# gabrielcheda/optimized-rag

Hardware: AMD Instinct MI355X
Metric: queries/sec + p50 retrieve+rerank latency, 1536-d top-k=20 (higher is better)
Workload: dtype f16 MFMA + block-scaled bf8 MFMA corrections (fp32 acc) in the cross-encoder; f16 MFMA pass + f64 rescore in the dense leg; f64 BM25 / RRF; 1 GPU; 1000000 docs x 1536-d + BM25 postings (2M-term Zipf vocabulary) + 224-token passage store; batch=256 queries: dense top-100 + BM25 top-100 + RRF -> top-100 -> ms-marco-MiniLM-L-6 cross-encoder (L=256, 25,600 pairs, seeded weights) -> top-20 (BASELINE.json configs[3]); corpus_rows=1000000, rows_per_gpu=1000000, batch_queries=256, pool=100, k=20, parallelism=one rag_retrieve_rerank_dev call per batch, exchange=single process

## Files before the change

### optimized-rag_amd/csrc/ce_mx.h

```cpp
#pragma once
#include "common.h"

typedef int mx_v8i __attribute__((ext_vector_type(8)));
typedef int mx_v4i __attribute__((ext_vector_type(4)));

#define MX_TM 384
#define MX_TN 128
#define MX_A_PLANE (MX_TM * 16)
#define MX_B_PLANE (MX_TN * 16)
#define MX_A_STAGE (6 * MX_A_PLANE)
#define MX_B_STAGE (6 * MX_B_PLANE)
#define MX_STAGE (MX_A_STAGE + MX_B_STAGE)
#define MX_STAGES 3
#define MX_LDS (MX_STAGES * MX_STAGE)
#ifndef MX_HI8_TRUNCATE
#define MX_LO_SCALE 2048.0f
#else
#define MX_LO_SCALE (2048.0f * 1.0928961748633879f)
#endif
#define MX_SCALE_A 116
#define MX_SCALE_B 127

__host__ __device__ __forceinline__ int mx_hi_off(int rows, int r, int e) {
    const int j = e >> 4, h = (e >> 2) & 1, i = ((e >> 3) & 1) * 4 + (e & 3);
// ... 258 lines not shown
    MX_STORE16(img + hh * MX_B_PLANE + trow * 16, ((mx_u4){hi[0][0], hi[0][1], hi[1][0], hi[1][1]}));
    MX_STORE16(img + (2 + hh) * MX_B_PLANE + trow * 16, ((mx_u4){hi[2][0], hi[2][1], hi[3][0], hi[3][1]}));
    MX_STORE16(img + (4 + hh) * MX_B_PLANE + trow * 16, ((mx_u4){lo[0], lo[2], lo[1], lo[3]}));
}

__global__ void mx_pack_weight_kernel(const float* __restrict__ w, int N, int K, char* __restrict__ out) {
    const int64_t i = (int64_t)blockIdx.x * blockDim.x + threadIdx.x;
    if (i >= (int64_t)N * K) return;
    const int n = (int)(i / K), k = (int)(i % K);
    const float x = w[i];
    const half_t hi = (half_t)x;
    const half_t l = (half_t)((x - (float)hi) * MX_LO_SCALE);
    char* img = out + ((size_t)(n / MX_TM) * (K >> 5) + (k >> 5)) * MX_A_STAGE;
    *reinterpret_cast<half_t*>(img + mx_hi_off(MX_TM, n % MX_TM, k & 31)) = hi;
    *reinterpret_cast<unsigned char*>(img + mx_lo_off(MX_TM, n % MX_TM, k & 31)) =
        (unsigned char)mx_e5m2_rn((unsigned)__builtin_bit_cast(unsigned short, l));
}

#define MX_EMB_ROWS 16
__global__ __launch_bounds__(256) void mx_embed_ln_kernel(const int32_t* __restrict__ ids, const int32_t* __restrict__ tt,
                                                           const float* __restrict__ word, const float* __restrict__ pos,
                                                           const float* __restrict__ type, const float* __restrict__ g,
                                                           const float* __restrict__ b, const int32_t* __restrict__ m_packed,
                                                           const int32_t* __restrict__ row_pair, const int32_t* __restrict__ pair_off,
                                                           int L, int vocab, float eps, char* __restrict__ x8) {
    constexpr int H = 384, NK = H / 32;
    __shared__ __attribute__((aligned(16))) char tile[NK * 6 * MX_EMB_ROWS * 16];
    const int lane = threadIdx.x & 63, wv = threadIdx.x >> 6;
    const int64_t base = (int64_t)blockIdx.x * MX_EMB_ROWS;
    const int n_rows = m_packed[0];
    if (base >= n_rows) return;
    const bool on = lane < H / 8;
    const int c = on ? lane : 0;
    const float4 g0 = *reinterpret_cast<const float4*>(g + c * 8), g1 = *reinterpret_cast<const float4*>(g + c * 8 + 4);
    const float4 b0 = *reinterpret_cast<const float4*>(b + c * 8), b1 = *reinterpret_cast<const float4*>(b + c * 8 + 4);
    const int j = (c >> 1) & 1, u = c & 1;
    char* const my = tile + (c >> 2) * 6 * MX_EMB_ROWS * 16;
#pragma unroll
    for (int r4 = 0; r4 < MX_EMB_ROWS / 4; ++r4) {
        const int rl = wv * (MX_EMB_ROWS / 4) + r4;
        const int64_t row = base + rl;
        if (row >= n_rows) break;
        const int pr = row_pair[row];
        const int p = (int)row - pair_off[pr];
        const size_t src = (size_t)pr * L + p;
        int id = ids[src];
        id = id < 0 ? 0 : (id >= vocab ? vocab - 1 : id);
        const int ty = tt[src] != 0;
        float v[8];
        {
            const float4* wp = reinterpret_cast<const float4*>(word + (size_t)id * H + c * 8);
            const float4* tp = reinterpret_cast<const float4*>(type + (size_t)ty * H + c * 8);
            const float4* pp = reinterpret_cast<const float4*>(pos + (size_t)p * H + c * 8);
#pragma unroll
            for (int q = 0; q < 2; ++q) {
                const float4 a = wp[q], t4 = tp[q], qq = pp[q];
                v[q * 4] = a.x + t4.x + qq.x; v[q * 4 + 1] = a.y + t4.y + qq.y; v[q * 4 + 2] = a.z + t4.z + qq.z; v[q * 4 + 3] = a.w + t4.w + qq.w;
            }
        }
        float s = 0.f;
#pragma unroll
        for (int i = 0; i < 8; ++i) s += on ? v[i] : 0.f;
#pragma unroll
        for (int o = 32; o > 0; o >>= 1) s += __shfl_xor(s, o);
        const float mean = s * (1.0f / H);
        float qd = 0.f;
#pragma unroll
// ... 4 lines not shown
        if (on) {
            mx_u2 h0, h1;
            unsigned l0, l1;
            mx_split4((v[0] - mean) * rstd * g0.x + b0.x, (v[1] - mean) * rstd * g0.y + b0.y, (v[2] - mean) * rstd * g0.z + b0.z,
                      (v[3] - mean) * rstd * g0.w + b0.w, h0, l0);
            mx_split4((v[4] - mean) * rstd * g1.x + b1.x, (v[5] - mean) * rstd * g1.y + b1.y, (v[6] - mean) * rstd * g1.z + b1.z,
                      (v[7] - mean) * rstd * g1.w + b1.w, h1, l1);
            char* o = my + rl * 16;
            *reinterpret_cast<mx_u2*>(o + (2 * j) * MX_EMB_ROWS * 16 + u * 8) = h0;
            *reinterpret_cast<mx_u2*>(o + (2 * j + 1) * MX_EMB_ROWS * 16 + u * 8) = h1;
            *reinterpret_cast<unsigned*>(o + 4 * MX_EMB_ROWS * 16 + u * 8 + j * 4) = l0;
            *reinterpret_cast<unsigned*>(o + 5 * MX_EMB_ROWS * 16 + u * 8 + j * 4) = l1;
        }
    }
    __syncthreads();
    const int trow0 = (int)(base & 127);
    char* const out = x8 + (size_t)(base >> 7) * NK * MX_B_STAGE + trow0 * 16;
    for (int i = threadIdx.x; i < NK * 6 * MX_EMB_ROWS; i += 256) {
        const int sp = i >> 4, r = i & (MX_EMB_ROWS - 1);
        if (base + r < n_rows) *reinterpret_cast<mx_u4*>(out + (size_t)sp * MX_B_PLANE + r * 16) = *reinterpret_cast<const mx_u4*>(tile + i * 16);
    }
}

__global__ void mx_gather_rows_kernel(const char* __restrict__ a, const char* __restrict__ b, const int32_t* __restrict__ pair_off, int P, int nk,
                                      char* __restrict__ a_out, char* __restrict__ b_out, int32_t* __restrict__ rows_out) {
    const int64_t i = (int64_t)blockIdx.x * blockDim.x + threadIdx.x;
    if (i == 0) rows_out[0] = P;
    const int per = nk * 6;
    if (i >= (int64_t)P * per) return;
    const int p = (int)(i / per), c = (int)(i % per), s = c / 6, pl = c % 6;
    const int64_t m = pair_off[p];
    const size_t src = ((size_t)(m >> 7) * nk + s) * MX_B_STAGE + (size_t)pl * MX_B_PLANE + (size_t)(m & 127) * 16;
    const size_t dst = ((size_t)(p >> 7) * nk + s) * MX_B_STAGE + (size_t)pl * MX_B_PLANE + (size_t)(p & 127) * 16;
    *reinterpret_cast<mx_u4*>(a_out + dst) = *reinterpret_cast<const mx_u4*>(a + src);
    if (b != nullptr) *reinterpret_cast<mx_u4*>(b_out + dst) = *reinterpret_cast<const mx_u4*>(b + src);
}

__device__ __forceinline__ float mx_load_elem(const char* __restrict__ x8, int64_t m, int k, int nk) {
    const char* img = x8 + mx_img_base(m, k, nk);
    const int trow = (int)(m & 127);
    return mx_join(*reinterpret_cast<const half_t*>(img + mx_hi_off(MX_TN, trow, k & 31)),
                   *reinterpret_cast<const unsigned char*>(img + mx_lo_off(MX_TN, trow, k & 31)));
}

struct mx_epi_qkv {
    half_t *qf16, *kf16, *vf16;
    size_t kv_plane;
    const float* bias;
    int m_tiles16;
    int ft_base;
    const int32_t* row_map;
    int n_map;
    __device__ __forceinline__ bool swap_for(int ft) const { return ft + ft_base == 2; }
    __device__ __forceinline__ void prepare(char* scratch) const { mx_stage_params(reinterpret_cast<float*>(scratch + MX_PARAM_OFF), bias, 3 * MX_TM); }
    __device__ __forceinline__ void operator()(f32x16 (&acc)[6], int tt, int ft_launch, bool swap, char* scratch) const {
        const float* const bias = reinterpret_cast<const float*>(scratch + MX_PARAM_OFF);
        const int ft = ft_launch + ft_base;
        const int lane = threadIdx.x & 63, wid = threadIdx.x >> 6, wm = wid >> 2, wn = wid & 3;
        const int li = lane & 31, hh = lane >> 5;
        const int m0 = tt * MX_TN + wn * 32;
        if (!swap) {
            half_t* dst = ft == 0 ? qf16 : kf16;
            int m = m0 + li;
            if (row_map != nullptr) {
                if (m >= n_map) return;
                m = row_map[m];
            }
#pragma unroll
            for (int b = 0; b < 6; ++b) {
                const int head = wm * 6 + b;
                half_t* tile = dst + (((size_t)head * m_tiles16 + (m >> 4)) * 64 + (m & 15)) * 8 + 4 * hh;
#pragma unroll
                for (int q = 0; q < 4; ++q) {
                    const float4 bv = *reinterpret_cast<const float4*>(bias + ft * MX_TM + head * 32 + 8 * q + 4 * hh);
                    const float v0 = acc[b][q * 4] + bv.x, v1 = acc[b][q * 4 + 1] + bv.y, v2 = acc[b][q * 4 + 2] + bv.z, v3 = acc[b][q * 4 + 3] + bv.w;
                    const half4 hi = {(half_t)v0, (half_t)v1, (half_t)v2, (half_t)v3};
                    const half4 lo = mx_resid4(hi, v0, v1, v2, v3);
                    __builtin_nontemporal_store(hi, reinterpret_cast<half4*>(tile + q * 128));
                    __builtin_nontemporal_store(lo, reinterpret_cast<half4*>(tile + q * 128 + kv_plane));
                }
            }
        } else {
#pragma unroll
            for (int b = 0; b < 6; ++b) {
                const int head = wm * 6 + b;
                const float bv = bias[2 * MX_TM + head * 32 + li];
#pragma unroll
                for (int q = 0; q < 4; ++q) {
                    const float v0 = acc[b][q * 4] + bv, v1 = acc[b][q * 4 + 1] + bv, v2 = acc[b][q * 4 + 2] + bv, v3 = acc[b][q * 4 + 3] + bv;
                    const half4 hi = {(half_t)v0, (half_t)v1, (half_t)v2, (half_t)v3};
                    const half4 lo = mx_resid4(hi, v0, v1, v2, v3);
                    half_t* o = vf16 + ((((size_t)head * m_tiles16 + (m0 >> 4) + (q >> 1)) * 2 + (li >> 4)) * 64 + (2 * (q & 1) + hh) * 16 + (li & 15)) * 4;
                    __builtin_nontemporal_store(hi, reinterpret_cast<half4*>(o));
                    __builtin_nontemporal_store(lo, reinterpret_cast<half4*>(o + kv_plane));
                }
            }
        }
    }
};

__device__ __forceinline__ float ce_gelu(float x) {
    const float z = fabsf(x) * 0.70710678118654752440f;
    const float t = __builtin_amdgcn_rcpf(fmaf(0.3275911f, z, 1.0f));
    float p = fmaf(1.061405429f, t, -1.453152027f);
    p = fmaf(p, t, 1.421413741f);
    p = fmaf(p, t, -0.284496736f);
    p = fmaf(p, t, 0.254829592f);
    const float e = __builtin_amdgcn_exp2f(-z * z * 1.4426950408889634f);
    const float erf_abs = fmaf(-p * t, e, 1.0f);
    return 0.5f * x * (1.0f + copysignf(erf_abs, x));
}
__device__ __forceinline__ float mx_gelu(float x) {
    const float z = fabsf(x) * 0.70710678118654752440f;
    const float t = __builtin_amdgcn_rcpf(fmaf(0.3275911f, z, 1.0f));
    float p = fmaf(1.061405429f, t, -1.453152027f);
// ... 123 lines not shown
```

### optimized-rag_amd/csrc/cross_encoder.hip

```cpp
#include "common.h"
#include "ce_mx.h"
#include <type_traits>

#include <cmath>
#include <cstdlib>
#include <cstring>

struct ce_chunk_bufs {
    dev_buf<int32_t> ids, tt, lens;
    dev_buf<int32_t> clen;
    dev_buf<int32_t> pair_off, row_pair, m_packed;
    dev_buf<int32_t> sid, stt;
    dev_buf<float> logits;
};

struct ce_ws_base {
    int pairs = 0, L = 0;
    int64_t tokens = 0;
    ce_chunk_bufs io;
    bool fits(int P, int L_) const { return P <= pairs && L_ == L; }
};
struct ce_split_ws : ce_ws_base {
    dev_buf<float> y32;
    dev_buf<half_t> x16, q16, kf16, vf16, ctx16, h16;
};
struct ce_mx_ws : ce_ws_base {
    dev_buf<char> x8, ctx8, h8;
    dev_buf<char> xc8, cc8, hc8;
    dev_buf<int32_t> m_cls;
    dev_buf<half_t> qf16, kf16, vf16;
};

struct ce_heads {
    int tok_dim = 0, tok_pad = 0;
// ... 302 lines not shown
                                               int hidden, float eps, int lane, half_t* __restrict__ o16) {
    float s = 0.f;
#pragma unroll
    for (int i = 0; i < PER; ++i) s += v[i];
#pragma unroll
    for (int o = 32; o > 0; o >>= 1) s += __shfl_xor(s, o);
    const float mean = s / (float)hidden;
    float q = 0.f;
#pragma unroll
    for (int i = 0; i < PER; ++i) { const float d = v[i] - mean; q += d * d; }
#pragma unroll
    for (int o = 32; o > 0; o >>= 1) q += __shfl_xor(q, o);
    const float rstd = 1.0f / sqrtf(q / (float)hidden + eps);
#pragma unroll
    for (int i = 0; i < PER; ++i) {
        const int c = lane + i * 64;
        const float y = (v[i] - mean) * rstd * g[c] + b[c];
        const half_t hi = (half_t)y;
        o16[SPLIT_IDX(c)] = hi;
        o16[SPLIT_IDX(c) + 32] = (half_t)(y - (float)hi);
    }
}

__global__ __launch_bounds__(1024) void ce_pack_scan_kernel(const int32_t* __restrict__ lens, int P, int L_in, int32_t* __restrict__ clen,
                                                             int32_t* __restrict__ pair_off, int32_t* __restrict__ m_packed) {
    __shared__ int part[1024];
    const int tid = threadIdx.x;
    const int per = (P + 1023) / 1024;
    const int b = tid * per, e = min(P, b + per);
    int s = 0;
    for (int p = b; p < e; ++p) s += (max(1, min(lens[p], L_in)) + 15) & ~15;
    part[tid] = s;
    __syncthreads();
    for (int o = 1; o < 1024; o <<= 1) {
        const int v = tid >= o ? part[tid - o] : 0;
        __syncthreads();
        part[tid] += v;
        __syncthreads();
    }
    int off = part[tid] - s;
    for (int p = b; p < e; ++p) {
        const int len = max(1, min(lens[p], L_in));
        clen[p] = len;
        pair_off[p] = off;
        off += (len + 15) & ~15;
    }
    if (tid == 1023) { pair_off[P] = part[1023]; m_packed[0] = part[1023]; }
}

__global__ void ce_pack_rows_kernel(const int32_t* __restrict__ pair_off, int P, int L, int64_t rows_total,
                                    int32_t* __restrict__ row_pair) {
    const int64_t i = (int64_t)blockIdx.x * blockDim.x + threadIdx.x;
    if (i < rows_total && i >= pair_off[P]) row_pair[i] = -1;
    if (i >= (int64_t)P * L) return;
    const int p = (int)(i / L), t = (int)(i % L);
    if (t < pair_off[p + 1] - pair_off[p]) row_pair[pair_off[p] + t] = p;
}

template <int PER>
__global__ __launch_bounds__(256) void ce_embed_ln_kernel(const int32_t* __restrict__ ids, const int32_t* __restrict__ tt,
                                                           const float* __restrict__ word, const float* __restrict__ pos,
                                                           const float* __restrict__ type, const float* __restrict__ g,
                                                           const float* __restrict__ b, const int32_t* __restrict__ m_packed,
                                                           const int32_t* __restrict__ row_pair, const int32_t* __restrict__ pair_off,
                                                           int L, int hidden, int vocab, int max_pos, float eps, half_t* __restrict__ x16) {
    const int lane = threadIdx.x & 63;
    const int64_t row = (int64_t)blockIdx.x * 4 + (threadIdx.x >> 6);
    if (row >= m_packed[0]) return;
    const int pr = row_pair[row];
    const int p = (int)row - pair_off[pr];
    const int pp = min(p, max_pos - 1);
    const size_t src = (size_t)pr * L + p;
    int id = ids[src];
    id = id < 0 ? 0 : (id >= vocab ? vocab - 1 : id);
    const int ty = tt[src] != 0;
    float v[PER];
#pragma unroll
    for (int i = 0; i < PER; ++i) {
        const int c = lane + i * 64;
// ... 12 lines not shown
    float v[PER];
#pragma unroll
    for (int i = 0; i < PER; ++i) v[i] = y32[tok * hidden + lane + i * 64];
    wave_layernorm<PER>(v, g, b, hidden, eps, lane, x16 + tok * 2 * hidden);
}

typedef uint32_t u32x4 __attribute__((ext_vector_type(4)));
typedef uint32_t u32x2 __attribute__((ext_vector_type(2)));
__device__ __forceinline__ uint32_t ce_pk(float a, float b) {
    return __builtin_bit_cast(uint32_t, __builtin_amdgcn_cvt_pkrtz(a, b));
}
__device__ __forceinline__ float ce_trunc10(float e) {
    return __builtin_bit_cast(float, __builtin_bit_cast(uint32_t, e) & 0xFFFFE000u);
}
__device__ __forceinline__ void ce_dma_at(const half_t* __restrict__ g, char* lds_uniform) {
    __builtin_amdgcn_global_load_lds((const __attribute__((address_space(1))) void*)g,
                                     (__attribute__((address_space(3))) void*)lds_uniform, 16, 0, 0);
}

template <int QB, bool MX = false, bool DIRECT = false>
__global__ __launch_bounds__(1024) void ce_attention_kernel(const half_t* __restrict__ q16,
                                                             const half_t* __restrict__ kf16, const half_t* __restrict__ vf16,
                                                             size_t kv_plane, const int32_t* __restrict__ lens,
                                                             const int32_t* __restrict__ pair_off, int L, int hidden,
                                                             int heads, int m_pad, half_t* __restrict__ ctx16, int max_qblocks = 1 << 20) {
    extern __shared__ __attribute__((aligned(16))) char smem[];
    const int lane = threadIdx.x & 63;
    const int wv = __builtin_amdgcn_readfirstlane(threadIdx.x >> 6), nwaves = blockDim.x >> 6;
    const int head = blockIdx.x, pair = blockIdx.y;
    const int len = max(1, min(lens[pair], L));
    const int fr = lane & 15, fq = lane >> 4;
    const int po = pair_off[pair], Lp = pair_off[pair + 1] - po;
    const int nt = Lp >> 4;
    const int nkb = (len + 31) >> 5;
    const size_t plane_b = (size_t)L * 64;
    const size_t t0 = ((size_t)head * (m_pad >> 4) + (po >> 4)) * 512;
    const char* const k_hi = DIRECT ? reinterpret_cast<const char*>(kf16 + t0) : smem;
    const char* const k_lo = DIRECT ? reinterpret_cast<const char*>(kf16 + t0 + kv_plane) : smem + plane_b;
    const char* const v_hi = DIRECT ? reinterpret_cast<const char*>(vf16 + t0) : smem + 2 * plane_b;
    const char* const v_lo = DIRECT ? reinterpret_cast<const char*>(vf16 + t0 + kv_plane) : smem + 3 * plane_b;
    if (!DIRECT) {
        char* const sk_hi = smem;
        char* const sk_lo = smem + plane_b;
        char* const sv_hi = smem + 2 * plane_b;
        char* const sv_lo = smem + 3 * plane_b;
        const size_t g0 = (((size_t)head * (m_pad >> 4) + (po >> 4)) * 64 + lane) * 8;
        for (int c = wv; c < nt; c += nwaves) {
            ce_dma_at(kf16 + g0 + (size_t)c * 512, sk_hi + c * 1024);
            ce_dma_at(kf16 + g0 + kv_plane + (size_t)c * 512, sk_lo + c * 1024);
            ce_dma_at(vf16 + g0 + (size_t)c * 512, sv_hi + c * 1024);
            ce_dma_at(vf16 + g0 + kv_plane + (size_t)c * 512, sv_lo + c * 1024);
        }
        if ((nt & 1) && wv == 0) {
            *reinterpret_cast<u32x4*>(sv_hi + nt * 1024 + lane * 16) = (u32x4){0u, 0u, 0u, 0u};
            *reinterpret_cast<u32x4*>(sv_lo + nt * 1024 + lane * 16) = (u32x4){0u, 0u, 0u, 0u};
// ... 8 lines not shown
        const int qb = (qb0 + b) * 16 < Lp ? qb0 + b : qb0;
        if (MX) {
            const half_t* qp = q16 + (((size_t)head * (m_pad >> 4) + (po >> 4) + qb) * 64 + lane) * 8;
            qh[b] = *reinterpret_cast<const half8*>(qp);
            ql[b] = *reinterpret_cast<const half8*>(qp + kv_plane);
        } else {
            const half_t* qp = q16 + (row0 + qb * 16 + fr) * (2 * hidden) + head * 64 + fq * 8;
            qh[b] = *reinterpret_cast<const half8*>(qp);
            ql[b] = *reinterpret_cast<const half8*>(qp + 32);
        }
    }
    f32x4 c0[QB], c1[QB];
    float mrun[QB], lsum[QB];
#pragma unroll
    for (int b = 0; b < QB; ++b) {
        c0[b] = (f32x4){0.f, 0.f, 0.f, 0.f};
        c1[b] = (f32x4){0.f, 0.f, 0.f, 0.f};
        mrun[b] = -INFINITY;
        lsum[b] = 0.f;
    }
    const float cs = (float)(0.17677669529663687 * 1.4426950408889634);
    if (!DIRECT) {
        asm volatile("s_waitcnt vmcnt(0)" ::: "memory");
        __syncthreads();
    }
    if (!has_rows) return;
    float ce_inf;
    asm volatile("s_mov_b32 %0, 0x7f800000" : "=s"(ce_inf));
#define CE_MAX2(a_, b_) __builtin_amdgcn_fmed3f(a_, b_, ce_inf)
    auto key_block = [&](const int kb, auto edge_c) {
        constexpr bool EDGE = decltype(edge_c)::value;
        const int fo = kb * 2048 + lane * 16;
        const half8 k0h = *reinterpret_cast<const half8*>(k_hi + fo), k1h = *reinterpret_cast<const half8*>(k_hi + fo + 1024);
        const half8 k0l = *reinterpret_cast<const half8*>(k_lo + fo), k1l = *reinterpret_cast<const half8*>(k_lo + fo + 1024);
        const int vo = kb * 2048 + lane * 8;
        const half4 a0h = *reinterpret_cast<const half4*>(v_hi + vo), a1h = *reinterpret_cast<const half4*>(v_hi + vo + 512);
        const half4 a0l = *reinterpret_cast<const half4*>(v_lo + vo), a1l = *reinterpret_cast<const half4*>(v_lo + vo + 512);
        half4 b0h = {}, b1h = {}, b0l = {}, b1l = {};
        if (!(DIRECT && EDGE && (nt & 1))) {
            b0h = *reinterpret_cast<const half4*>(v_hi + vo + 1024);
            b1h = *reinterpret_cast<const half4*>(v_hi + vo + 1536);
            b0l = *reinterpret_cast<const half4*>(v_lo + vo + 1024);
            b1l = *reinterpret_cast<const half4*>(v_lo + vo + 1536);
        }
        const half8 v0h = __builtin_shufflevector(a0h, b0h, 0, 1, 2, 3, 4, 5, 6, 7), v1h = __builtin_shufflevector(a1h, b1h, 0, 1, 2, 3, 4, 5, 6, 7);
        const half8 v0l = __builtin_shufflevector(a0l, b0l, 0, 1, 2, 3, 4, 5, 6, 7), v1l = __builtin_shufflevector(a1l, b1l, 0, 1, 2, 3, 4, 5, 6, 7);
#pragma unroll
        for (int b = 0; b < QB; ++b) {
            f32x4 z0 = {0.f, 0.f, 0.f, 0.f}, z1 = {0.f, 0.f, 0.f, 0.f};
            z0 = __builtin_amdgcn_mfma_f32_16x16x32_f16(k0l, qh[b], z0, 0, 0, 0);
            z1 = __builtin_amdgcn_mfma_f32_16x16x32_f16(k1l, qh[b], z1, 0, 0, 0);
            z0 = __builtin_amdgcn_mfma_f32_16x16x32_f16(k0h, ql[b], z0, 0, 0, 0);
            z1 = __builtin_amdgcn_mfma_f32_16x16x32_f16(k1h, ql[b], z1, 0, 0, 0);
            z0 = __builtin_amdgcn_mfma_f32_16x16x32_f16(k0h, qh[b], z0, 0, 0, 0);
            z1 = __builtin_amdgcn_mfma_f32_16x16x32_f16(k1h, qh[b], z1, 0, 0, 0);
            if (EDGE) {
#pragma unroll
                for (int r = 0; r < 4; ++r) {
                    if (kb * 32 + fq * 4 + r >= len) z0[r] = -INFINITY;
                    if (kb * 32 + 16 + fq * 4 + r >= len) z1[r] = -INFINITY;
                }
            }
            float mx = CE_MAX2(CE_MAX2(CE_MAX2(z0[0], z0[1]), CE_MAX2(z0[2], z0[3])), CE_MAX2(CE_MAX2(z1[0], z1[1]), CE_MAX2(z1[2], z1[3])));
            {
                float cp = mx;
                asm("s_nop 1\n\tv_permlane16_swap_b32 %0, %1" : "+v"(mx), "+v"(cp));
// ... 21 lines not shown
            const u32x4 ph_u = {ce_pk(eh[0], eh[1]), ce_pk(eh[2], eh[3]), ce_pk(eh[4], eh[5]), ce_pk(eh[6], eh[7])};
            const u32x4 pl_u = {ce_pk(e[0] - eh[0], e[1] - eh[1]), ce_pk(e[2] - eh[2], e[3] - eh[3]),
                                ce_pk(e[4] - eh[4], e[5] - eh[5]), ce_pk(e[6] - eh[6], e[7] - eh[7])};
            const half8 ph = __builtin_bit_cast(half8, ph_u), pl = __builtin_bit_cast(half8, pl_u);
            c0[b] = __builtin_amdgcn_mfma_f32_16x16x32_f16(v0l, ph, c0[b], 0, 0, 0);
            c1[b] = __builtin_amdgcn_mfma_f32_16x16x32_f16(v1l, ph, c1[b], 0, 0, 0);
            c0[b] = __builtin_amdgcn_mfma_f32_16x16x32_f16(v0h, pl, c0[b], 0, 0, 0);
            c1[b] = __builtin_amdgcn_mfma_f32_16x16x32_f16(v1h, pl, c1[b], 0, 0, 0);
            c0[b] = __builtin_amdgcn_mfma_f32_16x16x32_f16(v0h, ph, c0[b], 0, 0, 0);
            c1[b] = __builtin_amdgcn_mfma_f32_16x16x32_f16(v1h, ph, c1[b], 0, 0, 0);
        }
    };
    for (int kb = 0; kb + 1 < nkb; ++kb) key_block(kb, std::false_type{});
    key_block(nkb - 1, std::true_type{});
#undef CE_MAX2
#pragma unroll
    for (int b = 0; b < QB; ++b) {
        float l = lsum[b];
        l += __shfl_xor(l, 16);
        l += __shfl_xor(l, 32);
        const float inv = 1.0f / l;
        if ((qb0 + b) * 16 >= Lp || qb0 + b >= max_qblocks) break;
        if (MX) {
            const int64_t mrow = (int64_t)row0 + (qb0 + b) * 16 + fr;
            char* img = reinterpret_cast<char*>(ctx16) + mx_img_base(mrow, head * 32, hidden >> 5) + (int)(mrow & 127) * 16 + (fq >> 1) * 8;
            mx_u2 h0, h1;
            unsigned l0, l1;
            mx_split4(c0[b][0] * inv, c0[b][1] * inv, c0[b][2] * inv, c0[b][3] * inv, h0, l0);
            mx_split4(c1[b][0] * inv, c1[b][1] * inv, c1[b][2] * inv, c1[b][3] * inv, h1, l1);
            *reinterpret_cast<mx_u2*>(img + (fq & 1) * MX_B_PLANE) = h0;
            *reinterpret_cast<mx_u2*>(img + (2 + (fq & 1)) * MX_B_PLANE) = h1;
            *reinterpret_cast<mx_u2*>(img + (4 + (fq & 1)) * MX_B_PLANE) = (mx_u2){l0, l1};
            continue;
        }
        half_t* o = ctx16 + (row0 + (qb0 + b) * 16 + fr) * (2 * hidden) + head * 64 + fq * 4;
        store_split4(o, 32, c0[b][0] * inv, c0[b][1] * inv, c0[b][2] * inv, c0[b][3] * inv);
        store_split4(o + 16, 32, c1[b][0] * inv, c1[b][1] * inv, c1[b][2] * inv, c1[b][3] * inv);
    }
}

#define CE_A64_RESIDENT 0
#define CE_A64_DIRECT 1
#define CE_A64_STREAM 2
#define CE_A64_RING 4
#define CE_A64_SLOT 16384
template <int MODE>
__global__ __launch_bounds__(512) void ce_attention64_kernel(const half_t* __restrict__ q16, const half_t* __restrict__ kf16,
// ... 415 lines not shown
        if (c < tok_dim) out[(size_t)dst * tok_dim + c] = v[i] * sc;
    }
}

template <class T>
static int alloc_zeroed(rag_ctx* h, dev_buf<T>& b, size_t n, hipStream_t st) {
    if (int rc = b.alloc(h, n)) return rc;
    HIP_TRY(h, hipMemsetAsync(b, 0, n * sizeof(T), st));
    return RAG_OK;
}

template <class W>
static int ws_renew(rag_ctx* h, W& w, int P, int L, int out_width, hipStream_t st) {
    HIP_TRY(h, hipStreamSynchronize(st));
    w = W();
    const int64_t Mp = w.tokens = round_up((int64_t)P * L, 256);
    ce_chunk_bufs& c = w.io;
    int rc;
    if ((rc = c.ids.alloc(h, (size_t)Mp))) return rc;
    if ((rc = c.tt.alloc(h, (size_t)Mp))) return rc;
    if ((rc = c.lens.alloc(h, (size_t)P))) return rc;
    if ((rc = c.clen.alloc(h, (size_t)P))) return rc;
    if ((rc = c.pair_off.alloc(h, (size_t)P + 1))) return rc;
    if ((rc = c.row_pair.alloc(h, (size_t)Mp))) return rc;
    if ((rc = c.m_packed.alloc(h, 1))) return rc;
    if ((rc = c.sid.alloc(h, (size_t)P * L))) return rc;
    if ((rc = c.stt.alloc(h, (size_t)P * L))) return rc;
    return c.logits.alloc(h, (size_t)P * out_width);
}

void ce_free(rag_ctx* h) {
    delete h->ce;
    delete h->emb;
    h->ce = h->emb = nullptr;
}

static int up_f32(rag_ctx* h, const float* src, size_t n, dev_buf<float>& dst) {
    if (int rc = dst.alloc(h, n)) return rc;
    HIP_TRY(h, hipMemcpyAsync(dst, src, n * sizeof(float), hipMemcpyHostToDevice, h->stream));
    return RAG_OK;
}

static int up_weight(rag_ctx* h, std::vector<const float*> srcs, size_t rows_each, size_t cols, dev_buf<half_t>& dst16,
                     dev_buf<char>& dst8, bool mx) {
    const size_t n_each = rows_each * cols, total = n_each * srcs.size();
    const dim3 grid((unsigned)((total + 255) / 256));
    dev_buf<float> tmp;
// ... 102 lines not shown

static size_t kv_plane_halfs(int64_t Mp, size_t H) { return (size_t)Mp * H + 2048; }
static unsigned ce_gemm_grid(const rag_ctx* h) { return (unsigned)(h->n_cu >= 8 ? h->n_cu / 8 * 8 : 256); }

struct ce_chunk {
    const int32_t *ids, *tt, *lens;
    float* out;
    int P, L_in, L;
    float* lex = nullptr;
    float* tok = nullptr;
    const int64_t* row_off = nullptr;
    int64_t tok_cap = 0;
};

__global__ void ce_pad_tokens_kernel(const int32_t* __restrict__ in_ids, const int32_t* __restrict__ in_tt, int P, int L_in, int L,
                                     int32_t* __restrict__ ids, int32_t* __restrict__ tt) {
    const int64_t i = (int64_t)blockIdx.x * blockDim.x + threadIdx.x;
    if (i >= (int64_t)P * L) return;
    const int p = (int)(i / L), t = (int)(i % L);
    ids[i] = t < L_in ? in_ids[(size_t)p * L_in + t] : 0;
    tt[i] = t < L_in ? in_tt[(size_t)p * L_in + t] : 0;
}

static void chunk_prologue(const ce_ws_base& w, const ce_chunk& c, hipStream_t st) {
    const ce_chunk_bufs& io = w.io;
    launch(ce_pad_tokens_kernel, dim3((unsigned)(((int64_t)c.P * c.L + 255) / 256)), dim3(256), 0, st, c.ids, c.tt, c.P, c.L_in, c.L, io.ids, io.tt);
    launch(ce_pack_scan_kernel, dim3(1), dim3(1024), 0, st, c.lens, c.P, c.L_in, io.clen, io.pair_off, io.m_packed);
    launch(ce_pack_rows_kernel, dim3((unsigned)((w.tokens + 255) / 256)), dim3(256), 0, st, io.pair_off, c.P, c.L, w.tokens, io.row_pair);
}

template <int QB, bool MX>
static int launch_attention(rag_ctx* h, const rag_ce_model* m, const ce_ws_base& w, const half_t* q, const half_t* kf, const half_t* vf,
                            half_t* ctx, const ce_chunk& c, hipStream_t st, int max_qblocks = 1 << 20) {
    const int H = m->cfg.hidden, heads = m->cfg.heads, L = c.L;
    const size_t kv_plane = kv_plane_halfs(w.tokens, H);
    const dim3 grid(heads, c.P);
    if constexpr (MX)
        if (max_qblocks == 1) {
            launch(ce_attention_kernel<1, true, true>, grid, dim3(64), 0, st, q, kf, vf, kv_plane, w.io.clen, w.io.pair_off, L, H, heads,
                   (int)w.tokens, ctx, 1);
            return RAG_OK;
        }
    const int lds = L * 256;
    if (int rc = raise_lds(h, h->attr_ce_attn_lds[MX][QB], lds, ce_attention_kernel<QB, MX>)) return rc;
    launch(ce_attention_kernel<QB, MX>, grid, dim3(64 * (L / (16 * QB))), lds, st, q, kf, vf, kv_plane, w.io.clen, w.io.pair_off, L, H, heads,
           (int)w.tokens, ctx, max_qblocks);
    return RAG_OK;
}

#define CE_A64_STREAM_FROM 768
static int launch_attention64(rag_ctx* h, const rag_ce_model* m, const ce_split_ws& w, const ce_chunk& c, hipStream_t st) {
    const int H = m->cfg.hidden, L = c.L;
    const size_t kv_plane = kv_plane_halfs(w.tokens, H);
    const dim3 grid(m->cfg.heads, c.P), block(64 * (L / 32));
    const dim3 zgrid(m->cfg.heads, c.P, (L + 255) / 256);
    if (L <= 256) {
        const int lds = L * 512;
        if (int rc = raise_lds(h, h->attr_ce_attn64_lds, lds, ce_attention64_kernel<CE_A64_RESIDENT>)) return rc;
        launch(ce_attention64_kernel<CE_A64_RESIDENT>, grid, block, lds, st, w.q16, w.kf16, w.vf16, kv_plane, w.io.clen, w.io.pair_off, L, H,
               (int)w.tokens, w.ctx16);
    } else if (L > 512 && h->opt.ce_attn_stream >= 0 && (L >= CE_A64_STREAM_FROM || h->opt.ce_attn_stream > 0)) {
        const int lds = CE_A64_RING * CE_A64_SLOT;
        if (int rc = raise_lds(h, h->attr_ce_attn64s_lds, lds, ce_attention64_kernel<CE_A64_STREAM>)) return rc;
        launch(ce_attention64_kernel<CE_A64_STREAM>, zgrid, dim3(512), lds, st, w.q16, w.kf16, w.vf16, kv_plane, w.io.clen, w.io.pair_off, L, H,
               (int)w.tokens, w.ctx16);
    } else
        launch(ce_attention64_kernel<CE_A64_DIRECT>, zgrid, dim3(512), 0, st, w.q16, w.kf16, w.vf16, kv_plane, w.io.clen, w.io.pair_off, L, H,
               (int)w.tokens, w.ctx16);
    return RAG_OK;
// ... 50 lines not shown
    const int H = m->cfg.hidden;
    if (c.lex)
        launch(m3_lexical_kernel, dim3((unsigned)(((int64_t)c.P * c.L_in + 3) / 4)), dim3(256), 0, st, x16, io.pair_off, io.clen, c.P, c.L_in, H,
               hd.lex_w, hd.lex_b, c.lex);
    if (c.tok) {
        if (int rc = raise_lds(h, h->attr_m3_gemm_lds, CE_GEMM_LDS, ce_gemm_kernel<EPI_F32>)) return rc;
        launch(ce_gemm_kernel<EPI_F32>, dim3(ce_gemm_grid(h)), dim3(512), CE_GEMM_LDS, st, hd.tok_w, x16, hd.tok_pad, H, hd.tok_b, nullptr, hd.raw,
               nullptr, nullptr, nullptr, (size_t)0, H, m->cfg.heads, io.m_packed, (int)w.tokens);
        launch(m3_tok_scatter_kernel, dim3((unsigned)(((int64_t)c.P * c.L + 3) / 4)), dim3(256), 0, st, hd.raw, hd.tok_pad, hd.tok_dim, io.m_packed,
               io.row_pair, io.pair_off, io.clen, c.row_off, c.tok_cap, c.tok);
    }
    return RAG_OK;
}

static int ce_forward_chunk(rag_ctx* h, rag_ce_model* m, const ce_chunk& c, hipStream_t st) {
    ce_split_ws& w = m->split;
    const ce_chunk_bufs& io = w.io;
    const int H = m->cfg.hidden, F = m->cfg.ffn, P = c.P, L = c.L;
    const int64_t M = (int64_t)P * L;
    int rc;
    if ((rc = raise_lds(h, h->attr_ce_gemm_lds, CE_GEMM_LDS, ce_gemm_kernel<EPI_QKV>, ce_gemm_kernel<EPI_GELU>, ce_gemm_kernel<EPI_RESID>,
                        ce_gemm_kernel<EPI_QKV64>)))
        return rc;
    chunk_prologue(w, c, st);
    rc = per_lane_dispatch(h, H, [&](auto per) {
        launch(ce_embed_ln_kernel<decltype(per)::value>, dim3((unsigned)((M + 3) / 4)), dim3(256), 0, st, io.ids, io.tt, m->word, m->pos,
               m->type, m->emb_ln_g, m->emb_ln_b, io.m_packed, io.row_pair, io.pair_off, L, H, m->cfg.vocab_size, m->cfg.max_pos, (float)m->cfg.ln_eps, w.x16);
    });
    if (rc) return rc;
    for (const auto& ly : m->layers) {
        if (m->d_head == 64) {
            ce_gemm<EPI_QKV64>(h, m, st, ly.wqkv, w.x16, 3 * H, H, ly.bqkv, nullptr, nullptr, w.q16, w.kf16, w.vf16, kv_plane_halfs(w.tokens, H));
            rc = launch_attention64(h, m, w, c, st);
        } else {
            ce_gemm<EPI_QKV>(h, m, st, ly.wqkv, w.x16, 3 * H, H, ly.bqkv, nullptr, nullptr, w.q16, w.kf16, w.vf16, kv_plane_halfs(w.tokens, H));
            rc = L == 32 ? launch_attention<1, false>(h, m, w, w.q16, w.kf16, w.vf16, w.ctx16, c, st)
                         : launch_attention<2, false>(h, m, w, w.q16, w.kf16, w.vf16, w.ctx16, c, st);
        }
        if (rc) return rc;
        ce_gemm<EPI_RESID>(h, m, st, ly.wo, w.ctx16, H, H, ly.bo, w.x16, w.y32, nullptr);
        if ((rc = ce_layernorm(h, m, ly.ln1_g, ly.ln1_b, M, st))) return rc;
        ce_gemm<EPI_GELU>(h, m, st, ly.w1, w.x16, F, H, ly.b1, nullptr, nullptr, w.h16);
        ce_gemm<EPI_RESID>(h, m, st, ly.w2, w.h16, H, F, ly.b2, w.x16, w.y32, nullptr);
        if ((rc = ce_layernorm(h, m, ly.ln2_g, ly.ln2_b, M, st))) return rc;
    }
    if (m->embed) {
        if (c.out) launch(ce_meanpool_kernel<false>, dim3(P), dim3(256), 0, st, w.x16, io.pair_off, io.clen, L, H, m->normalize, m->pool_cls, c.out);
// ... 17 lines not shown
    if ((rc = alloc_zeroed(h, w.h8, rows * F * 3, st))) return rc;
    if ((rc = alloc_zeroed(h, w.xc8, cls_rows * H * 3, st))) return rc;
    if ((rc = alloc_zeroed(h, w.cc8, cls_rows * H * 3, st))) return rc;
    if ((rc = alloc_zeroed(h, w.hc8, cls_rows * F * 3, st))) return rc;
    if ((rc = w.m_cls.alloc(h, 1))) return rc;
    if ((rc = alloc_zeroed(h, w.qf16, 2 * kv, st))) return rc;
    if ((rc = alloc_zeroed(h, w.kf16, 2 * kv, st))) return rc;
    if ((rc = alloc_zeroed(h, w.vf16, 2 * kv, st))) return rc;
    w.pairs = P;
    w.L = L;
    return RAG_OK;
}

template <class EPI>
static void mx_gemm(rag_ctx* h, hipStream_t st, const char* W, const char* X, int nk, int n_ft, const int32_t* rows, EPI epi) {
    launch(mx_gemm_kernel<EPI>, dim3(ce_gemm_grid(h)), dim3(512), MX_KERNEL_LDS, st, W, X, nk, n_ft, rows, epi);
}

static void mx_qkv(rag_ctx* h, const rag_ce_model* m, const rag_ce_model::Layer& ly, hipStream_t st, int ft_base, int n_ft, const char* X,
                   const int32_t* rows, const int32_t* row_map = nullptr, int n_map = 0) {
    const ce_mx_ws& w = m->mx;
    const int nk = m->cfg.hidden / 32;
    mx_gemm(h, st, ly.wqkv8 + (size_t)ft_base * nk * MX_A_STAGE, X, nk, n_ft, rows,
            mx_epi_qkv{w.qf16, w.kf16, w.vf16, kv_plane_halfs(w.tokens, m->cfg.hidden), ly.bqkv, (int)(w.tokens >> 4), ft_base, row_map, n_map});
}

static void mx_layer_tail(rag_ctx* h, const rag_ce_model* m, const rag_ce_model::Layer& ly, hipStream_t st, const char* attn, char* x,
                          char* ffn, const int32_t* rows) {
    const int H = m->cfg.hidden, F = m->cfg.ffn;
    const float eps = (float)m->cfg.ln_eps;
    mx_gemm(h, st, ly.wo8, attn, H / 32, 1, rows, mx_epi_ln{x, ly.bo, ly.ln1_g, ly.ln1_b, eps});
    mx_gemm(h, st, ly.w18, x, H / 32, F / MX_TM, rows, mx_epi_gelu{ffn, ly.b1, F / 32});
    mx_gemm(h, st, ly.w28, ffn, F / 32, 1, rows, mx_epi_ln{x, ly.b2, ly.ln2_g, ly.ln2_b, eps});
}

static int mx_forward_chunk(rag_ctx* h, rag_ce_model* m, const ce_chunk& c, hipStream_t st) {
    ce_mx_ws& w = m->mx;
    const ce_chunk_bufs& io = w.io;
    const int H = m->cfg.hidden, P = c.P, L = c.L;
    int rc;
    if ((rc = raise_lds(h, h->attr_ce_mx_lds, MX_KERNEL_LDS, mx_gemm_kernel<mx_epi_qkv>, mx_gemm_kernel<mx_epi_gelu>, mx_gemm_kernel<mx_epi_ln>)))
        return rc;
    chunk_prologue(w, c, st);
    launch(mx_embed_ln_kernel, dim3((unsigned)(((int64_t)P * L + MX_EMB_ROWS - 1) / MX_EMB_ROWS)), dim3(256), 0, st, io.ids, io.tt, m->word,
           m->pos, m->type, m->emb_ln_g, m->emb_ln_b, io.m_packed, io.row_pair, io.pair_off, L, m->cfg.vocab_size, (float)m->cfg.ln_eps, w.x8);
    half_t* const ctx = reinterpret_cast<half_t*>(w.ctx8.get());
    const dim3 gather_grid((unsigned)(((int64_t)P * 72 + 255) / 256));
    bool cls_tail = false;
    for (int l = 0; l < m->cfg.layers; ++l) {
        const auto& ly = m->layers[l];
        cls_tail = !m->embed && l == m->cfg.layers - 1;
        if (cls_tail) {
            launch(mx_gather_rows_kernel, gather_grid, dim3(256), 0, st, w.x8, nullptr, io.pair_off, P, H / 32, w.xc8, nullptr, w.m_cls);
            mx_qkv(h, m, ly, st, 1, 2, w.x8, io.m_packed);
            mx_qkv(h, m, ly, st, 0, 1, w.xc8, w.m_cls, io.pair_off, P);
        } else
            mx_qkv(h, m, ly, st, 0, 3, w.x8, io.m_packed);
        const int qblocks = cls_tail ? 1 : 1 << 20;
        rc = L <= 256 ? launch_attention<1, true>(h, m, w, w.qf16, w.kf16, w.vf16, ctx, c, st, qblocks)
                      : launch_attention<2, true>(h, m, w, w.qf16, w.kf16, w.vf16, ctx, c, st, qblocks);
        if (rc) return rc;
        if (cls_tail) {
            launch(mx_gather_rows_kernel, gather_grid, dim3(256), 0, st, w.ctx8, nullptr, io.pair_off, P, H / 32, w.cc8, nullptr, w.m_cls);
            mx_layer_tail(h, m, ly, st, w.cc8, w.xc8, w.hc8, w.m_cls);
        } else
            mx_layer_tail(h, m, ly, st, w.ctx8, w.x8, w.h8, io.m_packed);
    }
    const char* const cls = cls_tail ? w.xc8 : w.x8;
    if (m->embed) {
        if (c.out)
            launch(ce_meanpool_kernel<true>, dim3(P), dim3(256), 0, st, reinterpret_cast<const half_t*>(w.x8.get()), io.pair_off, io.clen, L, H,
                   m->normalize, m->pool_cls, c.out);
        if (c.lex || c.tok) {
            launch(m3_mx_to_split_kernel, dim3((unsigned)(((int64_t)P * L * H + 255) / 256)), dim3(256), 0, st, w.x8, io.m_packed, H, m->heads.x16);
            if ((rc = heads_chunk(h, m, w, m->heads.x16, c, st))) return rc;
        }
    } else if (cls_tail && P >= 512)
        launch(mx_pool_classify_kernel, dim3((unsigned)((P + POOL_PB - 1) / POOL_PB)), dim3(256), 0, st, cls, m->wpT, m->bp, m->wc, m->bc, P, H, c.out);
    else
        launch(ce_pool_classify_kernel<true>, dim3(P), dim3(256), 0, st, reinterpret_cast<const half_t*>(cls), m->wp, m->bp, m->wc, m->bc,
               cls_tail ? nullptr : io.pair_off.get(), H, c.out);
    HIP_TRY(h, hipGetLastError());
    return RAG_OK;
}

static bool ce_use_mx(const rag_ctx* h, const rag_ce_model* m) {
    return m->mx_ok && (h->opt.ce_mx > 0 || (h->opt.ce_mx == 0 && m->mx_default));
}

static int heads_ensure_ws(rag_ctx* h, rag_ce_model* m, int64_t tokens, bool use_mx, bool tok, hipStream_t st) {
    ce_heads& hd = m->heads;
    const size_t H = m->cfg.hidden;
    int rc;
    if (use_mx && hd.x16_tokens != tokens) {
        HIP_TRY(h, hipStreamSynchronize(st));
        hd.x16_tokens = 0;
        if ((rc = alloc_zeroed(h, hd.x16, 2 * (size_t)tokens * H, st))) return rc;
        hd.x16_tokens = tokens;
    }
    if (tok && hd.raw_tokens != tokens) {
        HIP_TRY(h, hipStreamSynchronize(st));
        hd.raw_tokens = 0;
        if ((rc = hd.raw.alloc(h, (size_t)tokens * hd.tok_pad))) return rc;
        hd.raw_tokens = tokens;
// ... 198 lines not shown
```

Before: 1032 queries/sec.

## Pack cross-encoder token rows at 4-row granularity instead of 16 in MX path

```diff
diff --git a/optimized-rag_amd/csrc/ce_mx.h b/optimized-rag_amd/csrc/ce_mx.h
--- a/optimized-rag_amd/csrc/ce_mx.h
+++ b/optimized-rag_amd/csrc/ce_mx.h
@@ -304,7 +304,7 @@
                                                            const float* __restrict__ word, const float* __restrict__ pos,
                                                            const float* __restrict__ type, const float* __restrict__ g,
                                                            const float* __restrict__ b, const int32_t* __restrict__ m_packed,
-                                                           const int32_t* __restrict__ row_pair, const int32_t* __restrict__ pair_off,
+                                                           const int32_t* __restrict__ row_pair, const int32_t* __restrict__ row_off,
                                                            int L, int vocab, float eps, char* __restrict__ x8) {
     constexpr int H = 384, NK = H / 32;
     __shared__ __attribute__((aligned(16))) char tile[NK * 6 * MX_EMB_ROWS * 16];
@@ -324,7 +324,7 @@
         const int64_t row = base + rl;
         if (row >= n_rows) break;
         const int pr = row_pair[row];
-        const int p = (int)row - pair_off[pr];
+        const int p = (int)row - row_off[pr];
         const size_t src = (size_t)pr * L + p;
         int id = ids[src];
         id = id < 0 ? 0 : (id >= vocab ? vocab - 1 : id);
@@ -375,14 +375,14 @@
     }
 }
 
-__global__ void mx_gather_rows_kernel(const char* __restrict__ a, const char* __restrict__ b, const int32_t* __restrict__ pair_off, int P, int nk,
+__global__ void mx_gather_rows_kernel(const char* __restrict__ a, const char* __restrict__ b, const int32_t* __restrict__ row_off, int P, int nk,
                                       char* __restrict__ a_out, char* __restrict__ b_out, int32_t* __restrict__ rows_out) {
     const int64_t i = (int64_t)blockIdx.x * blockDim.x + threadIdx.x;
     if (i == 0) rows_out[0] = P;
     const int per = nk * 6;
     if (i >= (int64_t)P * per) return;
     const int p = (int)(i / per), c = (int)(i % per), s = c / 6, pl = c % 6;
-    const int64_t m = pair_off[p];
+    const int64_t m = row_off[p];
     const size_t src = ((size_t)(m >> 7) * nk + s) * MX_B_STAGE + (size_t)pl * MX_B_PLANE + (size_t)(m & 127) * 16;
     const size_t dst = ((size_t)(p >> 7) * nk + s) * MX_B_STAGE + (size_t)pl * MX_B_PLANE + (size_t)(p & 127) * 16;
     *reinterpret_cast<mx_u4*>(a_out + dst) = *reinterpret_cast<const mx_u4*>(a + src);
@@ -402,6 +402,7 @@
     const float* bias;
     int m_tiles16;
     int ft_base;
+    const int32_t* row_att;
     const int32_t* row_map;
     int n_map;
     __device__ __forceinline__ bool swap_for(int ft) const { return ft + ft_base == 2; }
@@ -412,17 +413,20 @@
         const int lane = threadIdx.x & 63, wid = threadIdx.x >> 6, wm = wid >> 2, wn = wid & 3;
         const int li = lane & 31, hh = lane >> 5;
         const int m0 = tt * MX_TN + wn * 32;
+        const int att = row_map == nullptr ? row_att[m0 + li] : -1;
         if (!swap) {
             half_t* dst = ft == 0 ? qf16 : kf16;
-            int m = m0 + li;
+            int m = att;
             if (row_map != nullptr) {
-                if (m >= n_map) return;
-                m = row_map[m];
-            }
+                if (m0 + li >= n_map) return;
+                m = row_map[m0 + li];
+            } else if (m < 0)
+                return;
+            const unsigned off = (unsigned)((m >> 4) * 512 + (m & 15) * 8 + 4 * hh);
 #pragma unroll
             for (int b = 0; b < 6; ++b) {
                 const int head = wm * 6 + b;
-                half_t* tile = dst + (((size_t)head * m_tiles16 + (m >> 4)) * 64 + (m & 15)) * 8 + 4 * hh;
+                half_t* tile = dst + (size_t)head * m_tiles16 * 512 + off;
 #pragma unroll
                 for (int q = 0; q < 4; ++q) {
                     const float4 bv = *reinterpret_cast<const float4*>(bias + ft * MX_TM + head * 32 + 8 * q + 4 * hh);
@@ -434,16 +438,23 @@
                 }
             }
         } else {
-#pragma unroll
-            for (int b = 0; b < 6; ++b) {
-                const int head = wm * 6 + b;
-                const float bv = bias[2 * MX_TM + head * 32 + li];
-#pragma unroll
-                for (int q = 0; q < 4; ++q) {
-                    const float v0 = acc[b][q * 4] + bv, v1 = acc[b][q * 4 + 1] + bv, v2 = acc[b][q * 4 + 2] + bv, v3 = acc[b][q * 4 + 3] + bv;
+            float bv[6];
+#pragma unroll
+            for (int b = 0; b < 6; ++b) bv[b] = bias[2 * MX_TM + (wm * 6 + b) * 32 + li];
+            int mq[4];
+#pragma unroll
+            for (int q = 0; q < 4; ++q) mq[q] = __shfl(att, 8 * q + 4 * hh);
+#pragma unroll
+            for (int q = 0; q < 4; ++q) {
+                const int ma = mq[q];
+                if (ma < 0) continue;
+                const unsigned off = (unsigned)((ma >> 4) * 512 + (li >> 4) * 256 + ((ma & 15) >> 2) * 64 + (li & 15) * 4);
+#pragma unroll
+                for (int b = 0; b < 6; ++b) {
+                    const float v0 = acc[b][q * 4] + bv[b], v1 = acc[b][q * 4 + 1] + bv[b], v2 = acc[b][q * 4 + 2] + bv[b], v3 = acc[b][q * 4 + 3] + bv[b];
                     const half4 hi = {(half_t)v0, (half_t)v1, (half_t)v2, (half_t)v3};
                     const half4 lo = mx_resid4(hi, v0, v1, v2, v3);
-                    half_t* o = vf16 + ((((size_t)head * m_tiles16 + (m0 >> 4) + (q >> 1)) * 2 + (li >> 4)) * 64 + (2 * (q & 1) + hh) * 16 + (li & 15)) * 4;
+                    half_t* o = vf16 + (size_t)(wm * 6 + b) * m_tiles16 * 512 + off;
                     __builtin_nontemporal_store(hi, reinterpret_cast<half4*>(o));
                     __builtin_nontemporal_store(lo, reinterpret_cast<half4*>(o + kv_plane));
                 }
diff --git a/optimized-rag_amd/csrc/cross_encoder.hip b/optimized-rag_amd/csrc/cross_encoder.hip
--- a/optimized-rag_amd/csrc/cross_encoder.hip
+++ b/optimized-rag_amd/csrc/cross_encoder.hip
@@ -9,7 +9,7 @@
 struct ce_chunk_bufs {
     dev_buf<int32_t> ids, tt, lens;
     dev_buf<int32_t> clen;
-    dev_buf<int32_t> pair_off, row_pair, m_packed;
+    dev_buf<int32_t> pair_off, row_off, row_pair, row_att, m_packed;
     dev_buf<int32_t> sid, stt;
     dev_buf<float> logits;
 };
@@ -358,39 +358,51 @@
     }
 }
 
-__global__ __launch_bounds__(1024) void ce_pack_scan_kernel(const int32_t* __restrict__ lens, int P, int L_in, int32_t* __restrict__ clen,
-                                                             int32_t* __restrict__ pair_off, int32_t* __restrict__ m_packed) {
-    __shared__ int part[1024];
+__global__ __launch_bounds__(1024) void ce_pack_scan_kernel(const int32_t* __restrict__ lens, int P, int L_in, int g, int32_t* __restrict__ clen,
+                                                             int32_t* __restrict__ pair_off, int32_t* __restrict__ row_off,
+                                                             int32_t* __restrict__ m_packed) {
+    __shared__ int part[1024], part_g[1024];
     const int tid = threadIdx.x;
     const int per = (P + 1023) / 1024;
     const int b = tid * per, e = min(P, b + per);
-    int s = 0;
-    for (int p = b; p < e; ++p) s += (max(1, min(lens[p], L_in)) + 15) & ~15;
+    int s = 0, sg = 0;
+    for (int p = b; p < e; ++p) {
+        const int len = max(1, min(lens[p], L_in));
+        s += (len + 15) & ~15;
+        sg += (len + g - 1) & ~(g - 1);
+    }
     part[tid] = s;
+    part_g[tid] = sg;
     __syncthreads();
     for (int o = 1; o < 1024; o <<= 1) {
-        const int v = tid >= o ? part[tid - o] : 0;
+        const int v = tid >= o ? part[tid - o] : 0, vg = tid >= o ? part_g[tid - o] : 0;
         __syncthreads();
         part[tid] += v;
+        part_g[tid] += vg;
         __syncthreads();
     }
-    int off = part[tid] - s;
+    int off = part[tid] - s, off_g = part_g[tid] - sg;
     for (int p = b; p < e; ++p) {
         const int len = max(1, min(lens[p], L_in));
         clen[p] = len;
         pair_off[p] = off;
+        row_off[p] = off_g;
         off += (len + 15) & ~15;
-    }
-    if (tid == 1023) { pair_off[P] = part[1023]; m_packed[0] = part[1023]; }
-}
-
-__global__ void ce_pack_rows_kernel(const int32_t* __restrict__ pair_off, int P, int L, int64_t rows_total,
-                                    int32_t* __restrict__ row_pair) {
+        off_g += (len + g - 1) & ~(g - 1);
+    }
+    if (tid == 1023) { pair_off[P] = part[1023]; row_off[P] = part_g[1023]; m_packed[0] = part_g[1023]; }
+}
+
+__global__ void ce_pack_rows_kernel(const int32_t* __restrict__ pair_off, const int32_t* __restrict__ row_off, int P, int L, int64_t rows_total,
+                                    int32_t* __restrict__ row_pair, int32_t* __restrict__ row_att) {
     const int64_t i = (int64_t)blockIdx.x * blockDim.x + threadIdx.x;
-    if (i < rows_total && i >= pair_off[P]) row_pair[i] = -1;
+    if (i < rows_total && i >= row_off[P]) row_pair[i] = row_att[i] = -1;
     if (i >= (int64_t)P * L) return;
     const int p = (int)(i / L), t = (int)(i % L);
-    if (t < pair_off[p + 1] - pair_off[p]) row_pair[pair_off[p] + t] = p;
+    if (t < row_off[p + 1] - row_off[p]) {
+        row_pair[row_off[p] + t] = p;
+        row_att[row_off[p] + t] = pair_off[p] + t;
+    }
 }
 
 template <int PER>
@@ -449,8 +461,9 @@
 __global__ __launch_bounds__(1024) void ce_attention_kernel(const half_t* __restrict__ q16,
                                                              const half_t* __restrict__ kf16, const half_t* __restrict__ vf16,
                                                              size_t kv_plane, const int32_t* __restrict__ lens,
-                                                             const int32_t* __restrict__ pair_off, int L, int hidden,
-                                                             int heads, int m_pad, half_t* __restrict__ ctx16, int max_qblocks = 1 << 20) {
+                                                             const int32_t* __restrict__ pair_off, const int32_t* __restrict__ row_off,
+                                                             int L, int hidden, int heads, int m_pad, half_t* __restrict__ ctx16,
+                                                             int max_qblocks = 1 << 20) {
     extern __shared__ __attribute__((aligned(16))) char smem[];
     const int lane = threadIdx.x & 63;
     const int wv = __builtin_amdgcn_readfirstlane(threadIdx.x >> 6), nwaves = blockDim.x >> 6;
@@ -458,6 +471,7 @@
     const int len = max(1, min(lens[pair], L));
     const int fr = lane & 15, fq = lane >> 4;
     const int po = pair_off[pair], Lp = pair_off[pair + 1] - po;
+    const int ro = row_off[pair], Lr = row_off[pair + 1] - ro;
     const int nt = Lp >> 4;
     const int nkb = (len + 31) >> 5;
     const size_t plane_b = (size_t)L * 64;
@@ -512,6 +526,11 @@
     const float cs = (float)(0.17677669529663687 * 1.4426950408889634);
     if (!DIRECT) {
         asm volatile("s_waitcnt vmcnt(0)" ::: "memory");
+        if (MX && Lr < Lp && wv == (nt - 1 < nwaves ? nt - 1 : nt - 1 - nwaves) && ((lane & 31) >> 3) >= ((Lr & 15) >> 2)) {
+            char* const sv = smem + 2 * plane_b + (nt - 1) * 1024 + lane * 16;
+            *reinterpret_cast<u32x4*>(sv) = (u32x4){0u, 0u, 0u, 0u};
+            *reinterpret_cast<u32x4*>(sv + plane_b) = (u32x4){0u, 0u, 0u, 0u};
+        }
         __syncthreads();
     }
     if (!has_rows) return;
@@ -524,14 +543,18 @@
         const half8 k0h = *reinterpret_cast<const half8*>(k_hi + fo), k1h = *reinterpret_cast<const half8*>(k_hi + fo + 1024);
         const half8 k0l = *reinterpret_cast<const half8*>(k_lo + fo), k1l = *reinterpret_cast<const half8*>(k_lo + fo + 1024);
         const int vo = kb * 2048 + lane * 8;
-        const half4 a0h = *reinterpret_cast<const half4*>(v_hi + vo), a1h = *reinterpret_cast<const half4*>(v_hi + vo + 512);
-        const half4 a0l = *reinterpret_cast<const half4*>(v_lo + vo), a1l = *reinterpret_cast<const half4*>(v_lo + vo + 512);
+        half4 a0h = *reinterpret_cast<const half4*>(v_hi + vo), a1h = *reinterpret_cast<const half4*>(v_hi + vo + 512);
+        half4 a0l = *reinterpret_cast<const half4*>(v_lo + vo), a1l = *reinterpret_cast<const half4*>(v_lo + vo + 512);
         half4 b0h = {}, b1h = {}, b0l = {}, b1l = {};
         if (!(DIRECT && EDGE && (nt & 1))) {
             b0h = *reinterpret_cast<const half4*>(v_hi + vo + 1024);
             b1h = *reinterpret_cast<const half4*>(v_hi + vo + 1536);
             b0l = *reinterpret_cast<const half4*>(v_lo + vo + 1024);
             b1l = *reinterpret_cast<const half4*>(v_lo + vo + 1536);
+        }
+        if (DIRECT && EDGE && MX) {
+            if (kb * 32 + fq * 4 >= Lr) a0h = a1h = a0l = a1l = (half4){};
+            if (kb * 32 + 16 + fq * 4 >= Lr) b0h = b1h = b0l = b1l = (half4){};
         }
         const half8 v0h = __builtin_shufflevector(a0h, b0h, 0, 1, 2, 3, 4, 5, 6, 7), v1h = __builtin_shufflevector(a1h, b1h, 0, 1, 2, 3, 4, 5, 6, 7);
         const half8 v0l = __builtin_shufflevector(a0l, b0l, 0, 1, 2, 3, 4, 5, 6, 7), v1l = __builtin_shufflevector(a1l, b1l, 0, 1, 2, 3, 4, 5, 6, 7);
@@ -599,7 +622,8 @@
         const float inv = 1.0f / l;
         if ((qb0 + b) * 16 >= Lp || qb0 + b >= max_qblocks) break;
         if (MX) {
-            const int64_t mrow = (int64_t)row0 + (qb0 + b) * 16 + fr;
+            if ((qb0 + b) * 16 + fr >= Lr) continue;
+            const int64_t mrow = (int64_t)ro + (qb0 + b) * 16 + fr;
             char* img = reinterpret_cast<char*>(ctx16) + mx_img_base(mrow, head * 32, hidden >> 5) + (int)(mrow & 127) * 16 + (fq >> 1) * 8;
             mx_u2 h0, h1;
             unsigned l0, l1;
@@ -1061,7 +1085,9 @@
     if ((rc = c.lens.alloc(h, (size_t)P))) return rc;
     if ((rc = c.clen.alloc(h, (size_t)P))) return rc;
     if ((rc = c.pair_off.alloc(h, (size_t)P + 1))) return rc;
+    if ((rc = c.row_off.alloc(h, (size_t)P + 1))) return rc;
     if ((rc = c.row_pair.alloc(h, (size_t)Mp))) return rc;
+    if ((rc = c.row_att.alloc(h, (size_t)Mp))) return rc;
     if ((rc = c.m_packed.alloc(h, 1))) return rc;
     if ((rc = c.sid.alloc(h, (size_t)P * L))) return rc;
     if ((rc = c.stt.alloc(h, (size_t)P * L))) return rc;
@@ -1210,11 +1236,12 @@
     tt[i] = t < L_in ? in_tt[(size_t)p * L_in + t] : 0;
 }
 
-static void chunk_prologue(const ce_ws_base& w, const ce_chunk& c, hipStream_t st) {
+static void chunk_prologue(const ce_ws_base& w, const ce_chunk& c, int g, hipStream_t st) {
     const ce_chunk_bufs& io = w.io;
     launch(ce_pad_tokens_kernel, dim3((unsigned)(((int64_t)c.P * c.L + 255) / 256)), dim3(256), 0, st, c.ids, c.tt, c.P, c.L_in, c.L, io.ids, io.tt);
-    launch(ce_pack_scan_kernel, dim3(1), dim3(1024), 0, st, c.lens, c.P, c.L_in, io.clen, io.pair_off, io.m_packed);
-    launch(ce_pack_rows_kernel, dim3((unsigned)((w.tokens + 255) / 256)), dim3(256), 0, st, io.pair_off, c.P, c.L, w.tokens, io.row_pair);
+    launch(ce_pack_scan_kernel, dim3(1), dim3(1024), 0, st, c.lens, c.P, c.L_in, g, io.clen, io.pair_off, io.row_off, io.m_packed);
+    launch(ce_pack_rows_kernel, dim3((unsigned)((w.tokens + 255) / 256)), dim3(256), 0, st, io.pair_off, io.row_off, c.P, c.L, w.tokens, io.row_pair,
+           io.row_att);
 }
 
 template <int QB, bool MX>
@@ -1225,14 +1252,14 @@
     const dim3 grid(heads, c.P);
     if constexpr (MX)
         if (max_qblocks == 1) {
-            launch(ce_attention_kernel<1, true, true>, grid, dim3(64), 0, st, q, kf, vf, kv_plane, w.io.clen, w.io.pair_off, L, H, heads,
-                   (int)w.tokens, ctx, 1);
+            launch(ce_attention_kernel<1, true, true>, grid, dim3(64), 0, st, q, kf, vf, kv_plane, w.io.clen, w.io.pair_off, w.io.row_off, L, H,
+                   heads, (int)w.tokens, ctx, 1);
             return RAG_OK;
         }
     const int lds = L * 256;
     if (int rc = raise_lds(h, h->attr_ce_attn_lds[MX][QB], lds, ce_attention_kernel<QB, MX>)) return rc;
-    launch(ce_attention_kernel<QB, MX>, grid, dim3(64 * (L / (16 * QB))), lds, st, q, kf, vf, kv_plane, w.io.clen, w.io.pair_off, L, H, heads,
-           (int)w.tokens, ctx, max_qblocks);
+    launch(ce_attention_kernel<QB, MX>, grid, dim3(64 * (L / (16 * QB))), lds, st, q, kf, vf, kv_plane, w.io.clen, w.io.pair_off, w.io.row_off, L,
+           H, heads, (int)w.tokens, ctx, max_qblocks);
     return RAG_OK;
 }
 
@@ -1329,7 +1356,7 @@
     if ((rc = raise_lds(h, h->attr_ce_gemm_lds, CE_GEMM_LDS, ce_gemm_kernel<EPI_QKV>, ce_gemm_kernel<EPI_GELU>, ce_gemm_kernel<EPI_RESID>,
                         ce_gemm_kernel<EPI_QKV64>)))
         return rc;
-    chunk_prologue(w, c, st);
+    chunk_prologue(w, c, 16, st);
     rc = per_lane_dispatch(h, H, [&](auto per) {
         launch(ce_embed_ln_kernel<decltype(per)::value>, dim3((unsigned)((M + 3) / 4)), dim3(256), 0, st, io.ids, io.tt, m->word, m->pos,
                m->type, m->emb_ln_g, m->emb_ln_b, io.m_packed, io.row_pair, io.pair_off, L, H, m->cfg.vocab_size, m->cfg.max_pos, (float)m->cfg.ln_eps, w.x16);
@@ -1393,7 +1420,8 @@
     const ce_mx_ws& w = m->mx;
     const int nk = m->cfg.hidden / 32;
     mx_gemm(h, st, ly.wqkv8 + (size_t)ft_base * nk * MX_A_STAGE, X, nk, n_ft, rows,
-            mx_epi_qkv{w.qf16, w.kf16, w.vf16, kv_plane_halfs(w.tokens, m->cfg.hidden), ly.bqkv, (int)(w.tokens >> 4), ft_base, row_map, n_map});
+            mx_epi_qkv{w.qf16, w.kf16, w.vf16, kv_plane_halfs(w.tokens, m->cfg.hidden), ly.bqkv, (int)(w.tokens >> 4), ft_base, w.io.row_att,
+                       row_map, n_map});
 }
 
 static void mx_layer_tail(rag_ctx* h, const rag_ce_model* m, const rag_ce_model::Layer& ly, hipStream_t st, const char* attn, char* x,
@@ -1412,9 +1440,9 @@
     int rc;
     if ((rc = raise_lds(h, h->attr_ce_mx_lds, MX_KERNEL_LDS, mx_gemm_kernel<mx_epi_qkv>, mx_gemm_kernel<mx_epi_gelu>, mx_gemm_kernel<mx_epi_ln>)))
         return rc;
-    chunk_prologue(w, c, st);
+    chunk_prologue(w, c, m->embed ? 16 : 4, st);
     launch(mx_embed_ln_kernel, dim3((unsigned)(((int64_t)P * L + MX_EMB_ROWS - 1) / MX_EMB_ROWS)), dim3(256), 0, st, io.ids, io.tt, m->word,
-           m->pos, m->type, m->emb_ln_g, m->emb_ln_b, io.m_packed, io.row_pair, io.pair_off, L, m->cfg.vocab_size, (float)m->cfg.ln_eps, w.x8);
+           m->pos, m->type, m->emb_ln_g, m->emb_ln_b, io.m_packed, io.row_pair, io.row_off, L, m->cfg.vocab_size, (float)m->cfg.ln_eps, w.x8);
     half_t* const ctx = reinterpret_cast<half_t*>(w.ctx8.get());
     const dim3 gather_grid((unsigned)(((int64_t)P * 72 + 255) / 256));
     bool cls_tail = false;
@@ -1422,7 +1450,7 @@
         const auto& ly = m->layers[l];
         cls_tail = !m->embed && l == m->cfg.layers - 1;
         if (cls_tail) {
-            launch(mx_gather_rows_kernel, gather_grid, dim3(256), 0, st, w.x8, nullptr, io.pair_off, P, H / 32, w.xc8, nullptr, w.m_cls);
+            launch(mx_gather_rows_kernel, gather_grid, dim3(256), 0, st, w.x8, nullptr, io.row_off, P, H / 32, w.xc8, nullptr, w.m_cls);
             mx_qkv(h, m, ly, st, 1, 2, w.x8, io.m_packed);
             mx_qkv(h, m, ly, st, 0, 1, w.xc8, w.m_cls, io.pair_off, P);
         } else
@@ -1432,7 +1460,7 @@
                       : launch_attention<2, true>(h, m, w, w.qf16, w.kf16, w.vf16, ctx, c, st, qblocks);
         if (rc) return rc;
         if (cls_tail) {
-            launch(mx_gather_rows_kernel, gather_grid, dim3(256), 0, st, w.ctx8, nullptr, io.pair_off, P, H / 32, w.cc8, nullptr, w.m_cls);
+            launch(mx_gather_rows_kernel, gather_grid, dim3(256), 0, st, w.ctx8, nullptr, io.row_off, P, H / 32, w.cc8, nullptr, w.m_cls);
             mx_layer_tail(h, m, ly, st, w.cc8, w.xc8, w.hc8, w.m_cls);
         } else
             mx_layer_tail(h, m, ly, st, w.ctx8, w.x8, w.h8, io.m_packed);
@@ -1450,7 +1478,7 @@
         launch(mx_pool_classify_kernel, dim3((unsigned)((P + POOL_PB - 1) / POOL_PB)), dim3(256), 0, st, cls, m->wpT, m->bp, m->wc, m->bc, P, H, c.out);
     else
         launch(ce_pool_classify_kernel<true>, dim3(P), dim3(256), 0, st, reinterpret_cast<const half_t*>(cls), m->wp, m->bp, m->wc, m->bc,
-               cls_tail ? nullptr : io.pair_off.get(), H, c.out);
+               cls_tail ? nullptr : io.row_off.get(), H, c.out);
     HIP_TRY(h, hipGetLastError());
     return RAG_OK;
 }
```

Result: faster. 1053 queries/sec, median of 6 (+2.0%).
